# PlakarLabs/plakar

Hardware: AMD Instinct MI355X
Metric: GiB/s chunked (device-resident, cut-points out) at 1/2/4/8 MI355X (higher is better)
Workload: dtype u8; 1 GPU; C1: 1x 1 GiB uniform random buffer per GPU (BASELINE configs[1]); bytes_per_gpu=1073741824, global_bytes=1073741824, buffers_per_gpu=1, chunk_params=FASTCDC min 65536 / normal 1048576 / max 4194304, gear=placeholder (v0.0.8 table unavailable; see DESIGN.md), parallelism=independent buffers, 1 rank per GPU x 1, no collective, streams=2

## Files before the change

### include/plakar_cdc.h

```cpp
#ifndef PLAKAR_CDC_H
#define PLAKAR_CDC_H

#include <stddef.h>
#include <stdint.h>

#ifdef __cplusplus
extern "C" {
#endif

#define CDC_ABI_VERSION 1

#define CDC_OK 0
#define CDC_EOF 1
#define CDC_NEED_DATA 2
#define CDC_E_INVALID (-1)
#define CDC_E_UNSUPPORTED (-2)
#define CDC_E_NOSPACE (-3)
#define CDC_E_DEVICE (-4)
#define CDC_E_NOMEM (-5)
#define CDC_E_NORMAL_SIZE (-6)
#define CDC_E_MIN_SIZE (-7)
#define CDC_E_MAX_SIZE (-8)
#define CDC_E_IO (-9)
#define CDC_E_NOT_INIT (-10)
// ... 310 lines not shown
                             uint64_t host_min_len, void *stream, uint64_t *host_chunks, uint64_t *host_bytes);
int cdc_chunk_entropy_device_async(int device, const uint32_t *d_hist, uint64_t rows, double *d_entropy,
                                   void *stream);

typedef struct cdc_stream cdc_stream;
int cdc_stream_new(const char *algorithm, const cdc_opts *opts, uint64_t window_bytes, int device,
                   cdc_stream **out);
int cdc_stream_buffer(cdc_stream *s, uint8_t **write_ptr, uint64_t *space);
int cdc_stream_commit(cdc_stream *s, uint64_t nbytes, int eof);
int cdc_stream_next(cdc_stream *s, const uint8_t **chunk, uint64_t *len);
void cdc_stream_free(cdc_stream *s);

typedef int64_t (*cdc_read_fn)(void *ctx, void *buf, uint64_t cap);
typedef struct cdc_chunker cdc_chunker;
int cdc_chunker_new(const char *algorithm, cdc_read_fn read, void *ctx, const cdc_opts *opts,
                    cdc_chunker **out);
int cdc_chunker_next(cdc_chunker *c, const uint8_t **chunk, uint64_t *len);
void cdc_chunker_free(cdc_chunker *c);

int cdc_set_debug_mode(int mode);

int cdc_set_maskl_index_mode(int mode);

int cdc_debug_maskl_state(int device, uint32_t *hint, uint64_t *groups);

int cdc_debug_stream_read(int device, const void *d_buf, uint64_t len, int reps, double best_us[3], double median_us[3],
                          void *stream);

int cdc_debug_set_digest_lanes(uint64_t lanes);

int cdc_profile_enable(int on);
int cdc_profile_collect(double *scan_ms, double *pipeline_ms, uint64_t *launches,
                        uint64_t *scan_bytes);

#ifdef __cplusplus
}
#endif
#endif
```

### plakar_amd/_lib.py

```python
import ctypes
import os
import sys
import warnings

_HERE = os.path.dirname(os.path.abspath(__file__))
LIB_PATH = os.environ.get("PLAKAR_CDC_LIB") or os.path.join(_HERE, "_lib", "libplakar_cdc.so")

CDC_OK = 0
CDC_EOF = 1
CDC_NEED_DATA = 2
CDC_E_INVALID = -1
CDC_E_UNSUPPORTED = -2
CDC_E_NOSPACE = -3
CDC_E_DEVICE = -4
CDC_E_NOMEM = -5
CDC_E_NORMAL_SIZE = -6
CDC_E_MIN_SIZE = -7
CDC_E_MAX_SIZE = -8
CDC_E_IO = -9
CDC_E_NOT_INIT = -10
CDC_E_NO_DEVICE = -11
CDC_E_AUTH = -12
CDC_E_CORRUPT = -13
CDC_E_MISMATCH = -14
# ... 251 lines not shown
    "cdc_archive_new": (ctypes.c_int, [ctypes.c_int, _P(cdc_archive_opts), _P(ctypes.c_void_p)]),
    "cdc_archive_add_packfile": (ctypes.c_int, [ctypes.c_void_p, ctypes.c_void_p, ctypes.c_uint64]),
    "cdc_archive_add_packfile_path": (ctypes.c_int, [ctypes.c_void_p, ctypes.c_char_p]),
    "cdc_archive_run": (ctypes.c_int, [ctypes.c_void_p, _P(cdc_archive_entry), ctypes.c_int, ctypes.c_char_p,
                                       ARCHIVE_DATA_FN, ARCHIVE_ENTRY_FN, ctypes.c_void_p, _P(cdc_archive_stats)]),
    "cdc_archive_free": (None, [ctypes.c_void_p]),
    "cdc_set_debug_mode": (ctypes.c_int, [ctypes.c_int]),
    "cdc_gear_is_placeholder": (ctypes.c_int, []),
    "cdc_set_maskl_index_mode": (ctypes.c_int, [ctypes.c_int]),
    "cdc_backup_run": (ctypes.c_int, [ctypes.c_int, _P(ctypes.c_char_p), ctypes.c_int, _P(cdc_backup_opts),
                                      BACKUP_FILE_FN, BACKUP_PACK_FN, ctypes.c_void_p, _P(cdc_backup_stats)]),
    "cdc_backup_new": (ctypes.c_int, [ctypes.c_int, _P(cdc_backup_opts), _P(ctypes.c_void_p)]),
    "cdc_backup_files": (ctypes.c_int, [ctypes.c_void_p, _P(ctypes.c_char_p), ctypes.c_int, BACKUP_FILE_FN,
                                        BACKUP_PACK_FN, ctypes.c_void_p, _P(cdc_backup_stats)]),
    "cdc_backup_free": (None, [ctypes.c_void_p]),
    "cdc_sha256": (ctypes.c_int, [ctypes.c_void_p, ctypes.c_uint64, ctypes.c_int, _P(ctypes.c_uint8)]),
    "cdc_sha256_accelerated": (ctypes.c_int, []),
    "cdc_chunk_entropy_device_async": (ctypes.c_int, [ctypes.c_int, ctypes.c_void_p, ctypes.c_uint64, ctypes.c_void_p,
                                                      ctypes.c_void_p]),
    "cdc_debug_maskl_state": (ctypes.c_int, [ctypes.c_int, _P(ctypes.c_uint32), _P(ctypes.c_uint64)]),
    "cdc_debug_stream_read": (ctypes.c_int, [ctypes.c_int, ctypes.c_void_p, ctypes.c_uint64, ctypes.c_int,
                                             ctypes.c_double * 3, ctypes.c_double * 3, ctypes.c_void_p]),
    "cdc_debug_set_digest_lanes": (ctypes.c_int, [ctypes.c_uint64]),
    "cdc_profile_enable": (ctypes.c_int, [ctypes.c_int]),
    "cdc_profile_collect": (ctypes.c_int, [_P(ctypes.c_double), _P(ctypes.c_double),
                                           _P(ctypes.c_uint64), _P(ctypes.c_uint64)]),
}

_lib = None


def lib():
    global _lib
    if _lib is None:
        if not os.path.exists(LIB_PATH):
            raise ImportError(
                f"libplakar_cdc.so not found at {LIB_PATH}: the HIP extension is required "
                "(build it with `python -m plakar_amd.build`); there is no CPU fallback")
        torch = sys.modules.get("torch")
        if torch is not None:
            try:
                torch.cuda.is_available()
            except Exception:
                pass
        L = ctypes.CDLL(LIB_PATH)
        for name, (res, args) in SIGNATURES.items():
# ... 55 lines not shown
```

### plakar_amd/csrc/cdc_api.cpp

```cpp
#include <hip/hip_runtime.h>

#include <algorithm>
#include <chrono>
#include <cerrno>
#include <cctype>
#include <cstdio>
#include <cstdlib>
#include <cstring>
#include <atomic>
#include <condition_variable>
#include <functional>
#include <mutex>
#include <string>
#include <thread>
#include <vector>

#include <fcntl.h>
#include <sys/stat.h>
#include <unistd.h>

#include "cdc_hostmem.h"
#include "cdc_internal.h"

using namespace cdc;
// ... 9 lines not shown
    hipEvent_t staged = nullptr;
    hipEvent_t done = nullptr;
    uint8_t *d_in() const { return in.as<uint8_t>(); }
    cdc_cut *d_cuts() const { return cuts.as<cdc_cut>(); }
    cdc_cut *h_cuts() const { return cuts_h.as<cdc_cut>(); }
    cdc_result *d_res() const { return res.as<cdc_result>(); }
    cdc_result *h_res() const { return res_h.as<cdc_result>(); }
};

constexpr int kBounces = 2;

struct DeviceCtx {
    int device = -1;
    uint64_t *d_gear = nullptr;
    hipStream_t stream = nullptr;
    hipStream_t copy = nullptr;
    std::mutex mu;
    Slot slot[2];
    PinBuf bounce[kBounces];
    hipEvent_t bounce_ev[kBounces] = {nullptr, nullptr};
    int next_bounce = 0;
    uint32_t *hint_h = nullptr, *hint_d = nullptr;
    std::atomic<uint64_t> groups{0};
};

struct Global {
    std::mutex mu;
    std::atomic<bool> init{false};
    bool placeholder_gear = true;
    uint64_t gear[256];
    uint64_t mask_s = kDefaultMaskS, mask_l = kDefaultMaskL;
    uint32_t cut_adj = 0;
    int debug_mode = 0;
    std::vector<DeviceCtx *> devs;
};

Global &G()
{
    static Global g;
    return g;
}

std::atomic<uint32_t> &maskl_index_mode()
{
    static std::atomic<uint32_t> m([] {
        const char *e = getenv("CDC_MASKL_INDEX");
// ... 95 lines not shown

int grow_bounce(DeviceCtx *c, uint64_t bytes)
{
    if (c->bounce[kBounces - 1].data() && bytes <= c->bounce[kBounces - 1].cap()) return CDC_OK;
    HIPCHK(hipStreamSynchronize(c->copy));
    for (int k = 0; k < kBounces; ++k) {
        if (!c->bounce[k].reserve(bytes)) return CDC_E_DEVICE;
        if (!c->bounce_ev[k]) HIPCHK(hipEventCreateWithFlags(&c->bounce_ev[k], hipEventDisableTiming));
        HIPCHK(hipEventRecord(c->bounce_ev[k], c->copy));
    }
    return CDC_OK;
}

Workspace carve(void *ws, const Plan &pl, const uint64_t *gear)
{
    char *b = static_cast<char *>(ws);
    Workspace W;
    W.runs = reinterpret_cast<uint64_t *>(b + pl.off_runs);
    W.w1_nodes = reinterpret_cast<uint64_t *>(b + pl.off_w1_nodes);
    W.xg = reinterpret_cast<uint64_t *>(b + pl.off_xg);
    W.sg = reinterpret_cast<uint64_t *>(b + pl.off_sg);
    W.flags = reinterpret_cast<uint32_t *>(b + pl.off_flags);
    W.tick = reinterpret_cast<uint32_t *>(b + pl.off_tick);
    W.gear = gear;
    W.runsL = reinterpret_cast<uint64_t *>(b + pl.off_runsL);
    W.validL = reinterpret_cast<uint32_t *>(b + pl.off_validL);
    return W;
}

int run_group(DeviceCtx *ctx, const DevParams &P, const void *const *data, const uint64_t *lens,
              int n, int final_, cdc_cut *const *cuts, const uint64_t *caps,
              cdc_result *const *res, void *ws, uint64_t ws_bytes, void *stream)
{
    Plan pl;
    int st = make_plan(lens, n, P, &pl);
    if (st != CDC_OK) return st;
    if (ws_bytes < pl.bytes) return CDC_E_INVALID;
    Batch B;
    std::memset(&B, 0, sizeof(B));
    B.nbufs = uint32_t(n);
    B.final_ = final_ ? 1u : 0u;
    B.total_segs = pl.total_segs;
    B.total_tasks = pl.total_tasks;
    B.seg = pl.seg;
    B.scan_lane = pl.scan_lane;
    B.persist = pl.persist;
// ... 13 lines not shown
        volatile uint32_t *hint = ctx->hint_h;
        if (hint && k % 1024 == 1023) *hint = 0u;
        const bool hinted = !hint || *hint != 0u;
        B.maskl_index = mli >= 2 || (mli == 1 && hinted) ? 1u : 0u;
        B.maskl_fused = P.fm_ok && (mli == 2 || (mli == 1 && hinted)) ? 1u : 0u;
        B.maskl_probe = mli == 1 && !hinted && k % 16 == 0 ? 1u : 0u;
        B.maskl_hint = ctx->hint_d;
    }
    B.force_fallback = G().debug_mode == 1 ? 1u : 0u;
    uint32_t segs = 0, tasks = 0;
    for (int i = 0; i < n; ++i) {
        BufDesc &D = B.b[i];
        D.data = static_cast<const uint8_t *>(data[i]);
        D.len = lens[i];
        D.out = cuts[i];
        D.cap = caps[i];
        D.res = res[i];
        D.seg_base = segs;
        D.nseg = uint32_t((lens[i] + B.seg - 1) / B.seg);
        D.task_base = tasks;
        segs += D.nseg;
        tasks += uint32_t((lens[i] + 64ull * pl.scan_lane - 1) / (64ull * pl.scan_lane));
    }
    const Workspace W = carve(ws, pl, ctx->d_gear);
    return launch_batch(B, P, W, stream);
}

int group_ws_bytes(const uint64_t *lens, int n, const DevParams &P, uint64_t *bytes)
{
    Plan pl;
    const int st = make_plan(lens, n, P, &pl);
    if (st != CDC_OK) return st;
    *bytes = pl.bytes;
    return CDC_OK;
}

int check_ready(int device, DeviceCtx **out)
{
    Global &g = G();
    if (!g.init.load(std::memory_order_acquire)) return CDC_E_NOT_INIT;
    for (auto *c : g.devs)
        if (c->device == device) {
            *out = c;
            return CDC_OK;
        }
    return CDC_E_INVALID;
}
// ... 413 lines not shown
    if (!algorithm || !opts) return CDC_E_INVALID;
    const std::string a = lower(algorithm);
    if (a != "fastcdc") return CDC_E_UNSUPPORTED;
    return validate_sizes(opts);
}

int cdc_set_debug_mode(int mode)
{
    G().debug_mode = mode;
    return CDC_OK;
}

int cdc_set_maskl_index_mode(int mode)
{
    if (mode < 0 || mode > 3) return CDC_E_INVALID;
    maskl_index_mode().store(uint32_t(mode), std::memory_order_relaxed);
    Global &g = G();
    std::lock_guard<std::mutex> lock(g.mu);
    for (DeviceCtx *c : g.devs)
        if (c && c->hint_h) *static_cast<volatile uint32_t *>(c->hint_h) = 0u;
    return CDC_OK;
}

int cdc_debug_set_digest_lanes(uint64_t lanes)
{
    cdc::g_digest_lanes = lanes;
    return CDC_OK;
}

int cdc_debug_maskl_state(int device, uint32_t *hint, uint64_t *groups)
{
    if (!hint || !groups) return CDC_E_INVALID;
    DeviceCtx *ctx = nullptr;
    const int st = check_ready(device, &ctx);
    if (st != CDC_OK) return st;
    if (hipSetDevice(device) != hipSuccess || hipDeviceSynchronize() != hipSuccess) return CDC_E_DEVICE;
    *hint = ctx->hint_h ? *static_cast<volatile uint32_t *>(ctx->hint_h) : 1u;
    *groups = ctx->groups.load(std::memory_order_relaxed);
    return CDC_OK;
}

int cdc_debug_stream_read(int device, const void *d_buf, uint64_t len, int reps, double best_us[3], double median_us[3],
                          void *stream)
{
    if (!d_buf || !best_us || !median_us) return CDC_E_INVALID;
    DeviceCtx *ctx = nullptr;
    const int st = check_ready(device, &ctx);
    if (st != CDC_OK) return st;
    if (hipSetDevice(device) != hipSuccess) return CDC_E_DEVICE;
    return launch_stream_read(d_buf, len, reps, best_us, median_us, stream);
}

int cdc_device_count(void)
{
    int n = 0;
    if (hipGetDeviceCount(&n) != hipSuccess) return 0;
    return n;
}

static void destroy_ctx(DeviceCtx *c)
{
    (void)hipSetDevice(c->device);
    if (c->stream) (void)hipStreamSynchronize(c->stream);
    (void)hipDeviceSynchronize();
    if (c->hint_h) (void)hipHostFree(c->hint_h);
    if (c->d_gear) (void)hipFree(c->d_gear);
    if (c->copy) (void)hipStreamSynchronize(c->copy);
    free_ctx_buffers(c);
    if (c->stream) (void)hipStreamDestroy(c->stream);
    if (c->copy) (void)hipStreamDestroy(c->copy);
    delete c;
}

static int create_ctx(int d, DeviceCtx **out)
{
    auto *c = new DeviceCtx();
    c->device = d;
    *out = nullptr;
    if (hipSetDevice(d) != hipSuccess || hipStreamCreateWithFlags(&c->stream, hipStreamNonBlocking) != hipSuccess ||
        hipMalloc(reinterpret_cast<void **>(&c->d_gear), 256 * sizeof(uint64_t)) != hipSuccess) {
        destroy_ctx(c);
        return CDC_E_DEVICE;
    }
    if (hipHostMalloc(reinterpret_cast<void **>(&c->hint_h), 64, hipHostMallocMapped | hipHostMallocCoherent) ==
        hipSuccess) {
        *c->hint_h = 0u;
        if (hipHostGetDevicePointer(reinterpret_cast<void **>(&c->hint_d), c->hint_h, 0) != hipSuccess) {
            (void)hipHostFree(c->hint_h);
            c->hint_h = c->hint_d = nullptr;
        }
    }
    *out = c;
    return CDC_OK;
}

int cdc_init(uint32_t dev_mask, const uint64_t gear[256], uint64_t mask_s, uint64_t mask_l,
             int cut_convention)
{
    Global &g = G();
    std::lock_guard<std::mutex> lock(g.mu);
    if (cut_convention != 0 && cut_convention != 1) return CDC_E_INVALID;
    uint64_t tab[256];
    if (gear)
// ... 978 lines not shown
```

### plakar_amd/csrc/cdc_internal.h

```cpp
#pragma once

#include <stddef.h>
#include <stdint.h>

#include <vector>

#include "plakar_cdc.h"

namespace cdc {

constexpr int kMaxBufsPerLaunch = 32;
constexpr int64_t kRowPending = -0x7FF0;
constexpr uint32_t kDbgForceAbort = 512;
constexpr uint32_t kForceAbortTicks = 20000;
constexpr uint32_t kRunCap = 4;
constexpr uint32_t kRecCntBits = 8, kRecEntBits = 14;
constexpr uint32_t kMaxScanLane = 1u << kRecEntBits;
constexpr uint32_t kMaxSegs = 1u << 22;
constexpr uint32_t kScanLaneBytes = 16384;
#ifndef CDC_WALK_WAVES
#define CDC_WALK_WAVES 4
#endif
constexpr uint32_t kWalkWavesPerWG = CDC_WALK_WAVES;
constexpr uint64_t kUndet = ~0ull;
// ... 24 lines not shown
    uint32_t final_;
    uint32_t total_segs, total_tasks;
    uint32_t force_fallback;
    uint32_t scan_lane;
    uint32_t debug;
    uint32_t spin_ticks;
    uint32_t maskl_index;
    uint32_t maskl_fused;
    uint32_t *maskl_hint;
    uint32_t maskl_probe;
    uint64_t seg;
    uint32_t persist;
    uint32_t scan_wgs;
    BufDesc b[kMaxBufsPerLaunch];
};

struct Workspace {
    uint64_t *runs;
    uint64_t *w1_nodes;
    uint64_t *xg;
    uint64_t *sg;
    uint32_t *flags;
    uint32_t *tick;
    const uint64_t *gear;
    uint64_t *runsL;
    uint32_t *validL;
};

struct Plan {
    uint64_t seg;
    uint32_t scan_lane;
    uint32_t total_segs, total_tasks;
    uint32_t persist, scan_wgs;
    size_t off_runs, off_w1_nodes, off_xg, off_sg, off_flags, off_tick, off_runsL, off_validL,
        bytes;
};

int make_plan(const uint64_t *lens, int nbufs, const DevParams &P, Plan *plan);
int launch_batch(const Batch &B, const DevParams &P, const Workspace &W, void *stream);
struct DigestBuf {
    const uint8_t *data;
    uint64_t len;
    const cdc_cut *cuts;
    uint64_t cap;
    const cdc_result *res;
    uint8_t *digests;
// ... 71 lines not shown
```

### plakar_amd/csrc/cdc_kernels.hip

```cpp
#include <hip/hip_ext.h>
#include <hip/hip_runtime.h>

#include <algorithm>
#include <mutex>
#include <type_traits>
#include <vector>

#include "cdc_hostmem.h"
#include "cdc_internal.h"

namespace cdc {

#ifndef CDC_SPIN_SLEEP
#define CDC_SPIN_SLEEP 1
#endif
constexpr int kSpinSleep = CDC_SPIN_SLEEP;

static constexpr uint64_t kNoHit = ~0ull;
static constexpr uint32_t kRawLaneBytes = 512;
static constexpr uint32_t kWarm = 64;

template <int NT, int COPIES = 32>
__device__ __forceinline__ void fill_gear_lds(uint64_t *tab, const uint64_t *gear, uint32_t sh = 0)
{
// ... 289 lines not shown
        for (int j = 0; j < 4; ++j) {
            const uint64_t r0 = r4 + 64u * j;
            if (r0 > rb) break;
            const uint64_t E = __ballot(rec_cnt(rec[j]) == 0);
            const uint32_t n = uint32_t(min(rb + 1 - r0, uint64_t(64)));
            const uint64_t Z = ~E & (n == 64 ? ~0ull : (1ull << n) - 1);
            const uint64_t below = Z & ((1ull << lane) - 1);
            const uint32_t prev = below ? lane - 1u - (63u - uint32_t(__builtin_clzll(below))) : cur + lane;
            const uint64_t r = r0 + lane;
            bool need = false;
            if (lane < n) {
                if ((E >> lane) & 1ull)
                    need = r >= ra && prev + 1 >= kc;
                else
                    need = prev >= kc && r + kMaskLSpill >= ra;
            }
            if (__ballot(need)) return true;
            cur = Z ? n - 1u - (63u - uint32_t(__builtin_clzll(Z))) : cur + n;
        }
    }
    return false;
}

template <bool kMaskL, bool kFused>
__device__ __forceinline__ void scan_task(const Batch &B, const DevParams &P, const Workspace &W, char *s_lds,
                                          const char *tab, uint32_t task, uint32_t lane, uint32_t wave,
                                          uint32_t laneoff);

template <bool kMaskL, bool kFused = false>
__device__ __forceinline__ void scan_body(const Batch &B, const DevParams &P, const Workspace &W)
{
    static_assert(!(kMaskL && kFused), "k_scan_f builds both indexes, from the MaskS records' side");
    __shared__ __attribute__((aligned(16)))
    char s_lds[kGearLdsBytes + kS2Waves * (kStageBytes + kQBytes) + (kFused ? kFlushTabBytes : 0u)];
    const uint32_t lane = threadIdx.x & 63u;
    const uint32_t wave = __builtin_amdgcn_readfirstlane(threadIdx.x >> 6);
    const uint32_t laneoff = (lane & 31u) << 3;
    const uint32_t task = blockIdx.x * kS2Waves + wave;
    bool act = true;
    if constexpr (kMaskL) {
        act = false;
        if (task < B.total_tasks) {
            uint32_t bb = 0;
            while (bb + 1 < B.nbufs && task >= B.b[bb + 1].task_base) ++bb;
            const BufDesc &Db = B.b[bb];
            const uint64_t t = task - Db.task_base;
            if (t * 64ull * B.scan_lane < Db.len) act = maskl_needed(B, P, W, Db, t, lane);
            if (lane == 0) W.validL[task] = act ? 1u : 0u;
        }
        if (!__syncthreads_or(act ? 1 : 0)) return;
        if (threadIdx.x == 0 && B.maskl_hint)
            __hip_atomic_store(B.maskl_hint, 1u, __ATOMIC_RELAXED, __HIP_MEMORY_SCOPE_SYSTEM);
    }
    if constexpr (!kMaskL) {
        const uint32_t gt = blockIdx.x * blockDim.x + threadIdx.x, nth = gridDim.x * blockDim.x;
        for (uint32_t i = gt; i < B.total_segs; i += nth) {
            W.xg[i] = 0ull;
            W.sg[i] = 0ull;
        }
        if (gt < kMaxBufsPerLaunch + 4)
            W.flags[gt] = gt == kLimitWord ? uint32_t(B.spin_ticks ? B.spin_ticks : kSpinLimit) : 0u;
        if (gt < 2) W.tick[gt] = 0u;
        if (gt < B.nbufs) B.b[gt].res->status = kRowPending;
        if (threadIdx.x == 0) dbg_ts(B, kTsScan + 4 * blockIdx.x);
    }
    uint32_t clk = 0;
    if (!kMaskL && (B.debug & kDbgClk) && blockIdx.x == 0 && threadIdx.x == 0) {
        clk = kTsClk + 4u * uint32_t(atomicAdd(reinterpret_cast<unsigned long long *>(&g_ts[kTsClkN]), 1ull) % kClkRecs);
        g_ts[clk] = __builtin_amdgcn_s_memrealtime();
        g_ts[clk + 1] = __builtin_amdgcn_s_memtime();
    }
    fill_gear_lds<kS2Waves * 64>(reinterpret_cast<uint64_t *>(s_lds), W.gear,
                                 kFused ? P.fm_sh : kMaskL ? P.fl_sh : P.fs_sh);
    if constexpr (kFused) {
        static_assert(kS2Waves * 64 >= 256, "one entry per thread");
        if (threadIdx.x < 256)
            reinterpret_cast<uint64_t *>(s_lds + kGearLdsBytes + kS2Waves * (kStageBytes + kQBytes))[threadIdx.x] =
                W.gear[threadIdx.x] << P.fs_sh;
    }
    __syncthreads();
    if (!kMaskL && threadIdx.x == 0) {
        dbg_ts(B, kTsScan + 4 * blockIdx.x + 1);
        if (blockIdx.x < 4096)
            dbg_ts(B, kTsHw + blockIdx.x,
                   uint64_t(__builtin_amdgcn_s_getreg(20 | (0 << 6) | (15 << 11))) << 32 |
                       uint32_t(__builtin_amdgcn_s_getreg(4 | (0 << 6) | (31 << 11))));
    }
    const char *tab = s_lds;
    if (!act) return;
    const bool persist = !kMaskL && B.persist != 0;
    auto next_task = [&]() { return wave_ticket(W.tick + 2); };
    for (uint32_t cur = persist ? next_task() : task;;) {
        if (cur >= B.total_tasks) break;
        scan_task<kMaskL, kFused>(B, P, W, s_lds, tab, cur, lane, wave, laneoff);
        if (!persist) break;
        cur = next_task();
    }
    if (clk && threadIdx.x == 0) {
        g_ts[clk + 2] = __builtin_amdgcn_s_memrealtime();
        g_ts[clk + 3] = __builtin_amdgcn_s_memtime();
    }
}

template <bool kMaskL, bool kFused>
__device__ __forceinline__ void scan_task(const Batch &B, const DevParams &P, const Workspace &W, char *s_lds,
                                          const char *tab, uint32_t task, uint32_t lane, uint32_t wave,
                                          uint32_t laneoff)
{
    uint32_t b = 0;
    while (b + 1 < B.nbufs && task >= B.b[b + 1].task_base) ++b;
    const BufDesc &D = B.b[b];

    const uint64_t sl = B.scan_lane;
    const uint64_t ub = reinterpret_cast<uint64_t>(D.data);
    const uint64_t lo_ok = ub & ~15ull, hi_ok = (ub + D.len + 15) & ~15ull;
    const uint64_t seg0 = uint64_t(task - D.task_base) * 64u;
    if (seg0 * sl >= D.len) return;
    const int64_t s = int64_t((seg0 + lane) * sl);
    constexpr uint32_t kLead = 128u;
    const uint32_t T = uint32_t((sl + kLead + (ub & 15u) + kStage - 1u) / kStage);
    const uint64_t wb = ((ub + seg0 * sl) & ~15ull) - kLead;
    const uint64_t base = wb > lo_ok ? wb : lo_ok;
    const uint64_t limw = hi_ok - 16u - base;
    const uint32_t lim = limw > 0x7FFFFFFFull ? 0x7FFFFFFFu : uint32_t(limw);
    const uint32_t ring = uint32_t(reinterpret_cast<uintptr_t>(s_lds)) + kGearLdsBytes + wave * kStageBytes;
    static_assert(kStage == 64 && kL == 4, "pair staging: 64-B stages, one slot");
    const uint32_t half = lane >> 5;
    const uint32_t row = lane & 31u, swz = (row >> 1) & 7u;
    uint32_t offi[4];
    uint32_t om = 0;
#pragma unroll
    for (uint32_t j = 0; j < 4; ++j) {
        const uint32_t r = 8u * j + lane / 8u;
        const uint32_t k = (lane % 8u) ^ ((r >> 1) & 7u);
        const uint32_t o = uint32_t((((ub + (seg0 + r) * sl) & ~15ull) - kLead + 16u * k) - base);
        om = max(om, o);
        offi[j] = o - 1024u * j;
    }
    const uint64_t om0 = scan_wave_max(om);
    const uint64_t half_step = 32ull * sl;
    auto issue = [&](auto PC, uint32_t u, auto FC) {
        constexpr uint32_t Q = decltype(PC)::value;
        constexpr bool kFast = decltype(FC)::value;
        const uint64_t adv = uint64_t(kStage) * (u - Q) + (Q ? half_step : 0ull);
#ifdef CDC_DIAG_NO_DMA
        return;
#endif
        if (kFast || om0 + adv <= uint64_t(lim)) {
#ifdef CDC_DIAG_L2
            dma_stage_imm(lo_ok + ((base + adv - lo_ok) & 0x7FFF0ull), ring, offi);
#else
            dma_stage_imm(base + adv, ring, offi);
#endif
        } else {
            uint32_t eff[4];
#pragma unroll
            for (uint32_t j = 0; j < 4; ++j) eff[j] = min(offi[j] + 1024u * j + uint32_t(adv), lim);
            dma_stage(base, ring, eff);
        }
    };
    const char *rowp = s_lds + kGearLdsBytes + wave * kStageBytes + row * 128u;
    auto load_row = [&](uint4 (&first)[4], uint4 (&second)[4]) {
#ifdef CDC_DIAG_NO_ROW
        asm volatile("" : "+v"(first[0].x), "+v"(second[0].x));
        return;
#endif
#pragma unroll
        for (uint32_t g = 0; g < 4; ++g) first[g] = *reinterpret_cast<const uint4 *>(rowp + 16u * (g ^ swz));
#pragma unroll
        for (uint32_t g = 0; g < 4; ++g) second[g] = *reinterpret_cast<const uint4 *>(rowp + 16u * ((g + 4) ^ swz));
    };
    const uint32_t TT = T + 1;
    const int32_t lag = int32_t(kStage * half);
    const uint32_t vhi = to_vgpr(kFused ? P.fm_mi : kMaskL ? P.fl_hi : P.fs_hi);
    const uint32_t xlo = kMaskL ? P.fl_lo : P.fs_lo, xhi = kMaskL ? P.fl_hi : P.fs_hi;
    const int64_t rel0 = int64_t(((ub + uint64_t(s)) & ~15ull) - kLead) - int64_t(ub);
    using C0 = std::integral_constant<uint32_t, 0>;
    using C1 = std::integral_constant<uint32_t, 1>;
    using Gen = std::integral_constant<bool, false>;
    using Steady = std::integral_constant<bool, true>;

    uint4 A[4] = {}, Bv[4] = {};
#ifdef CDC_DIAG_WAITS
    uint64_t wsum = 0;
    uint32_t nrc = 0;
    const uint64_t tk0 = __builtin_amdgcn_s_memtime();
    const uint64_t rt0 = __builtin_amdgcn_s_memrealtime();
#endif
    static_assert(kLead >= 2 * kStage, "stage 0 must be pure warm-up for both halves");
    issue(C0{}, 0, Gen{});
    wait_vmcnt<0>();
    if (half == 0) load_row(A, Bv);
    asm volatile("s_waitcnt lgkmcnt(0)" ::: "memory");
    if (1 < TT) issue(C1{}, 1, Gen{});
    if (1 < TT) {
        wait_vmcnt<0>();
        if (half == 1) load_row(Bv, A);
        asm volatile("s_waitcnt lgkmcnt(0)" ::: "memory");
        if (2 < TT) issue(C0{}, 2, Gen{});
    }
    uint64_t gv[2][16];
#pragma unroll
    for (int k = 0; k < 16; ++k) gv[0][k] = lds_gear(tab, gear_addr(laneoff, word_of(Bv[0], k >> 2), k));
    uint64_t fp = 0;
    uint64_t rec = 0;
    uint64_t recL = 0;
    const int32_t rr0 = int32_t(rel0 - s) - lag;
    uint64_t *const qf = reinterpret_cast<uint64_t *>(s_lds + kGearLdsBytes + kS2Waves * kStageBytes + wave * kQBytes);
    uint32_t *const qm = reinterpret_cast<uint32_t *>(qf + kQCap);
    static_assert(kQCap == 64, "one flush pass: item j in lane j");
    uint32_t qn = 0;
    const char *const ftab = s_lds + kGearLdsBytes + kS2Waves * (kStageBytes + kQBytes);
    auto rgear = [&](const uint4 &d, int k) -> uint64_t {
        if constexpr (kFused)
            return lds_gear(ftab, __builtin_amdgcn_ubfe(word_of(d, k >> 2), uint32_t(k & 3) * 8u, 8u) << 3);
        else
            return lds_gear(tab, gear_addr(laneoff, word_of(d, k >> 2), k));
    };
    auto flush = [&]() {
        {
            const bool v = lane < qn;
            const uint32_t meta = qm[v ? lane : 0u];
            const uint32_t owner = meta >> 24;
            const int32_t r0 = int32_t(meta & 0xFFFFFFu) - 256;
            const int64_t so = int64_t((seg0 + owner) * sl);
            const int32_t ln = so < int64_t(D.len) ? int32_t(min(int64_t(sl), int64_t(D.len) - so)) : 0;
            const uint64_t a = ub + uint64_t(so + r0);
            auto clamp16 = [&](uint64_t x) { return min(max(x, lo_ok), hi_ok - 16u); };
            const uint4 d0 = gload16(clamp16(a)), d1 = gload16(clamp16(a + 16u));
            uint64_t f = 0;
            if constexpr (kFused) {
                uint4 dw[4];
#pragma unroll
                for (int h = 0; h < 4; ++h) dw[h] = gload16(clamp16(a - 64u + 16u * uint32_t(h)));
#pragma unroll
                for (int k = 0; k < 64; ++k) f = (f << 1) + rgear(dw[k >> 4], k & 15);
            } else {
                f = qf[v ? lane : 0u];
            }
            uint32_t miss = 0, missL = 0;
#pragma unroll
            for (int k = 0; k < 32; ++k) {
                f = (f << 1) + rgear(k < 16 ? d0 : d1, k & 15);
                miss |= min(key_of(f, xlo, xhi), 1u) << k;
                if constexpr (kFused) missL |= min(key_of(f, P.fm_llo, P.fm_lhi), 1u) << k;
            }
            const int32_t lo = r0 < 0 ? -r0 : 0, hi = ln - r0;
            uint32_t vm = lo >= 32 ? 0u : (0xFFFFFFFFu << lo);
            vm &= hi >= 32 ? 0xFFFFFFFFu : (hi <= 0 ? 0u : (1u << hi) - 1u);
// ... 40 lines not shown
            if ((gi & 1) == 0) {
                f0 = fp;
                acc = 0xFFFFFFFFu;
            }
#pragma unroll
            for (int q = 0; q < 4; ++q) {
#pragma unroll
                for (int k = 4 * q; k < 4 * q + 4; k += 2) {
                    const uint32_t a0 = gear_addr(laneoff, word_of(nx, k >> 2), k);
                    fp = (fp << 1) + cg[k];
                    ng[k] = lds_gear(tab, a0);
                    const uint32_t k0 = uint32_t(fp >> 32) & vhi;
                    const uint32_t a1 = gear_addr(laneoff, word_of(nx, (k + 1) >> 2), k + 1);
                    fp = (fp << 1) + cg[k + 1];
                    ng[k + 1] = lds_gear(tab, a1);
                    acc = umin3(acc, k0, uint32_t(fp >> 32) & vhi);
                    __builtin_amdgcn_sched_barrier(0);
                }
                __builtin_amdgcn_sched_barrier(0);
                if (q == 1 && gi + 1 == kGroups && (kSteady || t + 2 < TT)) {
                    asm volatile("s_waitcnt lgkmcnt(8)" ::: "memory");
                    issue(PC, t + 2, SC);
                    __builtin_amdgcn_sched_barrier(0);
                }
            }
            if (gi & 1) {
#ifndef CDC_DIAG_NO_RECHECK
                const uint64_t fm = __ballot(acc == 0);
#ifdef CDC_DIAG_WAITS
                nrc += fm ? 1u : 0u;
#endif
                if (fm) [[unlikely]] {
                    const uint32_t nq = uint32_t(__popcll(fm));
                    if (qn + nq > kQCap) flush();
                    if (acc == 0) {
                        const uint32_t idx =
                            qn + __builtin_amdgcn_mbcnt_hi(uint32_t(fm >> 32), __builtin_amdgcn_mbcnt_lo(uint32_t(fm), 0u));
                        const int32_t r0 = rr0 + int32_t(kStage * t + 16u * (gi - 1));
                        if constexpr (!kFused) qf[idx] = f0;
                        qm[idx] = uint32_t(r0 + 256) | (lane << 24);
                    }
                    qn += nq;
                }
#else
                rec += acc == 0 ? 1u : 0u;
#endif
            }
        }
    };
    if (1 < TT) stage(C1{}, Gen{}, 1, Bv, A);
    const int64_t room = int64_t(lim) - int64_t(om0) - int64_t(half_step);
    const int64_t tf = room >= 128 ? room / 64 - 1 : 0;
    const uint32_t t_steady = uint32_t(max<int64_t>(2, min<int64_t>(int64_t(TT) - 3, tf)));
    uint32_t t = 2;
    for (; t < t_steady; t += 2) {
        stage(C0{}, Steady{}, t, A, Bv);
        stage(C1{}, Steady{}, t + 1, Bv, A);
    }
    for (; t < TT; t += 2) {
        stage(C0{}, Gen{}, t, A, Bv);
        if (t + 1 < TT) stage(C1{}, Gen{}, t + 1, Bv, A);
    }
    if (qn) flush();
    if (s < int64_t(D.len)) (kMaskL ? W.runsL : W.runs)[64ull * D.task_base + seg0 + lane] = rec;
    if constexpr (kFused) {
        if (s < int64_t(D.len)) W.runsL[64ull * D.task_base + seg0 + lane] = recL;
        if (lane == 0) W.validL[task] = 1u;
    }
    if (!kMaskL && lane == 0) dbg_ts(B, kTsScan + 4 * blockIdx.x + 2 + (wave & 1));
#ifdef CDC_DIAG_WAITS
    if (lane == 0 && 8 * task + 7 < 8 * 16384) {
        uint64_t *o = g_ts + kTsRes + 8 * task;
        o[0] = wsum;
        o[1] = __builtin_amdgcn_s_memtime() - tk0;
        o[2] = rt0;
        o[3] = __builtin_amdgcn_s_memrealtime();
        o[4] = __builtin_amdgcn_s_getreg(4 | (0 << 6) | (31 << 11));
        o[5] = __builtin_amdgcn_s_getreg(20 | (0 << 6) | (15 << 11));
        o[6] = nrc;
        o[7] = wave;
    }
#endif
}

#ifndef CDC_SCAN_LB
#define CDC_SCAN_LB (kS2Waves * 64)
#endif
__global__ __launch_bounds__(CDC_SCAN_LB) void k_scan(const Batch B, const DevParams P, const Workspace W)
{
    scan_body<false>(B, P, W);
}

__global__ __launch_bounds__(kS2Waves * 64) void k_scan_l(const Batch B, const DevParams P, const Workspace W)
{
    scan_body<true>(B, P, W);
}

__global__ __launch_bounds__(CDC_SCAN_LB) void k_scan_f(const Batch B, const DevParams P, const Workspace W)
{
    scan_body<false, true>(B, P, W);
}

constexpr uint32_t kProbeWaves = 4;

__global__ __launch_bounds__(kProbeWaves * 64) void k_maskl_probe(const Batch B, const DevParams P, const Workspace W)
// ... 1086 lines not shown
            B.b[i].res->ncuts = 0;
            B.b[i].res->consumed = 0;
            B.b[i].res->needed = 0;
            if (B.total_tasks) settle_row(B.b[i].res, CDC_OK);
            else B.b[i].res->status = CDC_OK;
        }
    }
}

#ifdef CDC_RESOLVE_WAVES_PER_EU
#define CDC_RESOLVE_ATTR __attribute__((amdgpu_waves_per_eu(CDC_RESOLVE_WAVES_PER_EU)))
#else
#define CDC_RESOLVE_ATTR
#endif
__global__ CDC_RESOLVE_ATTR __launch_bounds__(kWalkWavesPerWG * 64) void k_resolve(const Batch B, const DevParams P, const Workspace W)
{
    __builtin_amdgcn_s_setprio(3);
    __shared__ uint64_t s_tab[256 * kWCopies];
    __shared__ uint64_t s_grec[kWalkWavesPerWG][kGRecs];
    __shared__ uint64_t s_gx[kWalkWavesPerWG][kGExtra];
    __shared__ uint32_t s_ticket;
    const uint32_t wave = threadIdx.x >> 6, lane = threadIdx.x & 63u;
    if (threadIdx.x == 0) s_ticket = __hip_atomic_fetch_add(W.tick, 1u, __ATOMIC_RELAXED, __HIP_MEMORY_SCOPE_AGENT);
    fill_gear_lds<kWalkWavesPerWG * 64, kWCopies>(s_tab, W.gear);
    __syncthreads();
    if (blockIdx.x == 0 && wave == 0) write_empty_rows(B, lane);
    const uint32_t g = uint32_t(__builtin_amdgcn_readfirstlane(s_ticket)) * kWalkWavesPerWG + wave;
    if (g < B.total_segs)
        resolve_segment(B, P, W, g, reinterpret_cast<const char *>(s_tab), graph_lds(s_grec[wave], s_gx[wave]));
}

constexpr uint32_t kStreamThreads = 256;

__global__ __launch_bounds__(kStreamThreads) void k_stream_read(const uint4 *p, uint64_t n16, uint32_t *sink)
{
    const uint64_t stride = uint64_t(gridDim.x) * kStreamThreads;
    uint64_t i = uint64_t(blockIdx.x) * kStreamThreads + threadIdx.x;
    uint32_t x = 0;
    for (; i + 3 * stride < n16; i += 4 * stride) {
        const uint4 a = p[i], b = p[i + stride], c = p[i + 2 * stride], d = p[i + 3 * stride];
        x ^= a.x ^ a.y ^ a.z ^ a.w ^ b.x ^ b.y ^ b.z ^ b.w ^ c.x ^ c.y ^ c.z ^ c.w ^ d.x ^ d.y ^ d.z ^ d.w;
    }
    for (; i < n16; i += stride) {
        const uint4 a = p[i];
        x ^= a.x ^ a.y ^ a.z ^ a.w;
    }
// ... 189 lines not shown
    if (!g_prof_on) return false;
    if (!g_prof_pool.empty()) {
        r = g_prof_pool.back();
        g_prof_pool.pop_back();
    } else if (hipEventCreate(&r.e0) != hipSuccess || hipEventCreate(&r.e1) != hipSuccess ||
               hipEventCreate(&r.e2) != hipSuccess) {
        return false;
    }
    r.scan_bytes = bytes;
    return true;
}

int launch_batch(const Batch &B, const DevParams &P, const Workspace &W, void *stream)
{
    hipStream_t st = reinterpret_cast<hipStream_t>(stream);
    if (B.nbufs == 0) return CDC_OK;
    uint64_t bytes = 0;
    for (uint32_t i = 0; i < B.nbufs; ++i) bytes += B.b[i].len;
    ProfRec pr;
    const bool prof = prof_begin(pr, bytes);
    const uint32_t need_wgs = (B.total_tasks + kS2Waves - 1) / kS2Waves;
    const dim3 sgrid(B.persist && B.scan_wgs < need_wgs ? B.scan_wgs : need_wgs), sblock(kS2Waves * 64);
    const bool fused = B.maskl_index && B.maskl_fused;
    if (B.persist && B.total_tasks > 0 && hipMemsetAsync(W.tick + 2, 0, 4, st) != hipSuccess) return CDC_E_DEVICE;
    if (B.total_tasks == 0) {
        if (prof) {
            (void)hipEventRecord(pr.e0, st);
            (void)hipEventRecord(pr.e1, st);
        }
    } else if (prof) {
        if (fused)
            hipExtLaunchKernelGGL(k_scan_f, sgrid, sblock, 0, st, pr.e0, pr.e1, 0, B, P, W);
        else
            hipExtLaunchKernelGGL(k_scan, sgrid, sblock, 0, st, pr.e0, pr.e1, 0, B, P, W);
    } else if (fused) {
        hipLaunchKernelGGL(k_scan_f, sgrid, sblock, 0, st, B, P, W);
    } else {
        hipLaunchKernelGGL(k_scan, sgrid, sblock, 0, st, B, P, W);
    }
#ifdef CDC_DIAG_SCAN_ONLY
    if (prof) {
        std::lock_guard<std::mutex> lk(g_prof_mu);
        (void)hipEventRecord(pr.e2, st);
        g_prof_live.push_back(pr);
    }
    return hipGetLastError() == hipSuccess ? CDC_OK : CDC_E_DEVICE;
#endif
// ... 88 lines not shown
```

### plakar_amd/device.py

```python
import ctypes

import torch

from . import _lib
from ._lib import check, ensure_init, lib


def _opts_c(opts):
    return _lib.cdc_opts(opts.MinSize, opts.NormalSize, opts.MaxSize, 0)


class DeviceBatch:

    def __init__(self, tensors, opts, final=True, device=None):
        ensure_init()
        if not tensors:
            raise ValueError("no buffers")
        self.tensors = list(tensors)
        for t in self.tensors:
            if t.dtype != torch.uint8 or not t.is_cuda or not t.is_contiguous():
                raise ValueError("expected contiguous uint8 CUDA tensors")
        self.device = self.tensors[0].device.index if device is None else device
        self.opts = opts
        self.final = 1 if final else 0
# ... 31 lines not shown
            ncuts, consumed, status, needed = (int(x) for x in r[i])
            check(status, f"buffer {i}")
            c = self.cuts[i][:ncuts].clone()
            c[:, 1] &= 0xFFFFFFFF
            out.append(c)
        return out, r


def chunk_device(tensors, opts, final=True):
    b = DeviceBatch(tensors, opts, final=final)
    b.launch()
    cuts, _ = b.results()
    return cuts


def set_debug_mode(mode):
    lib().cdc_set_debug_mode(int(mode))


def set_maskl_index_mode(mode):
    check(lib().cdc_set_maskl_index_mode(int(mode)))


def maskl_state(device=0):
    hint, groups = ctypes.c_uint32(), ctypes.c_uint64()
    check(lib().cdc_debug_maskl_state(int(device), ctypes.byref(hint), ctypes.byref(groups)))
    return hint.value, groups.value
```

Measured before the change: 5153 GiB/s.

## Prefetch next persistent scan task's DMA during current task tail and drop tick memset

Restructures the persistent scan loop so each wave claims its next task ticket during the current task's tail. It issues that task's first DMA stages before the flush and run writeback, which hides per-task warm-up latency. The scan ticket counter moves to a per-stream device slot that a later kernel resets, removing a hipMemsetAsync launch per call. The cost is more complex control flow, descriptor state carried across tasks, and a small per-stream lookup table. It also adds a debug setter for scan tasks per wave.

```diff
diff --git a/include/plakar_cdc.h b/include/plakar_cdc.h
--- a/include/plakar_cdc.h
+++ b/include/plakar_cdc.h
@@ -356,6 +356,8 @@
 
 int cdc_set_maskl_index_mode(int mode);
 
+int cdc_debug_set_scan_tasks_per_wave(int k);
+
 int cdc_debug_maskl_state(int device, uint32_t *hint, uint64_t *groups);
 
 int cdc_debug_stream_read(int device, const void *d_buf, uint64_t len, int reps, double best_us[3], double median_us[3],
diff --git a/plakar_amd/_lib.py b/plakar_amd/_lib.py
--- a/plakar_amd/_lib.py
+++ b/plakar_amd/_lib.py
@@ -297,6 +297,7 @@
     "cdc_debug_stream_read": (ctypes.c_int, [ctypes.c_int, ctypes.c_void_p, ctypes.c_uint64, ctypes.c_int,
                                              ctypes.c_double * 3, ctypes.c_double * 3, ctypes.c_void_p]),
     "cdc_debug_set_digest_lanes": (ctypes.c_int, [ctypes.c_uint64]),
+    "cdc_debug_set_scan_tasks_per_wave": (ctypes.c_int, [ctypes.c_int]),
     "cdc_profile_enable": (ctypes.c_int, [ctypes.c_int]),
     "cdc_profile_collect": (ctypes.c_int, [_P(ctypes.c_double), _P(ctypes.c_double),
                                            _P(ctypes.c_uint64), _P(ctypes.c_uint64)]),
diff --git a/plakar_amd/csrc/cdc_api.cpp b/plakar_amd/csrc/cdc_api.cpp
--- a/plakar_amd/csrc/cdc_api.cpp
+++ b/plakar_amd/csrc/cdc_api.cpp
@@ -55,6 +55,22 @@
     int next_bounce = 0;
     uint32_t *hint_h = nullptr, *hint_d = nullptr;
     std::atomic<uint64_t> groups{0};
+    static constexpr int kTickStreams = 16, kTickStride = 32;
+    uint32_t *scan_ticks = nullptr;
+    std::mutex tick_mu;
+    std::vector<void *> tick_streams;
+    uint32_t *scan_tick_of(void *stream)
+    {
+        if (!scan_ticks || stream == static_cast<void *>(hipStreamPerThread)) return nullptr;
+        std::lock_guard<std::mutex> lk(tick_mu);
+        size_t i = 0;
+        while (i < tick_streams.size() && tick_streams[i] != stream) ++i;
+        if (i == tick_streams.size()) {
+            if (i >= size_t(kTickStreams)) return nullptr;
+            tick_streams.push_back(stream);
+        }
+        return scan_ticks + i * kTickStride;
+    }
 };
 
 struct Global {
@@ -196,6 +212,8 @@
     W.sg = reinterpret_cast<uint64_t *>(b + pl.off_sg);
     W.flags = reinterpret_cast<uint32_t *>(b + pl.off_flags);
     W.tick = reinterpret_cast<uint32_t *>(b + pl.off_tick);
+    W.scan_tick = W.tick + 2;
+    W.scan_tick_armed = 0u;
     W.gear = gear;
     W.runsL = reinterpret_cast<uint64_t *>(b + pl.off_runsL);
     W.validL = reinterpret_cast<uint32_t *>(b + pl.off_validL);
@@ -255,7 +273,11 @@
         segs += D.nseg;
         tasks += uint32_t((lens[i] + 64ull * pl.scan_lane - 1) / (64ull * pl.scan_lane));
     }
-    const Workspace W = carve(ws, pl, ctx->d_gear);
+    Workspace W = carve(ws, pl, ctx->d_gear);
+    if (uint32_t *tk = ctx->scan_tick_of(stream)) {
+        W.scan_tick = tk;
+        W.scan_tick_armed = 1u;
+    }
     return launch_batch(B, P, W, stream);
 }
 
@@ -715,6 +737,13 @@
     return CDC_OK;
 }
 
+int cdc_debug_set_scan_tasks_per_wave(int k)
+{
+    if (k < -1 || k > 64) return CDC_E_INVALID;
+    cdc::t_scan_tpw = k;
+    return CDC_OK;
+}
+
 int cdc_debug_set_digest_lanes(uint64_t lanes)
 {
     cdc::g_digest_lanes = lanes;
@@ -758,6 +787,7 @@
     (void)hipDeviceSynchronize();
     if (c->hint_h) (void)hipHostFree(c->hint_h);
     if (c->d_gear) (void)hipFree(c->d_gear);
+    if (c->scan_ticks) (void)hipFree(c->scan_ticks);
     if (c->copy) (void)hipStreamSynchronize(c->copy);
     free_ctx_buffers(c);
     if (c->stream) (void)hipStreamDestroy(c->stream);
@@ -772,6 +802,12 @@
     *out = nullptr;
     if (hipSetDevice(d) != hipSuccess || hipStreamCreateWithFlags(&c->stream, hipStreamNonBlocking) != hipSuccess ||
         hipMalloc(reinterpret_cast<void **>(&c->d_gear), 256 * sizeof(uint64_t)) != hipSuccess) {
+        destroy_ctx(c);
+        return CDC_E_DEVICE;
+    }
+    const size_t tick_bytes = size_t(DeviceCtx::kTickStreams) * DeviceCtx::kTickStride * sizeof(uint32_t);
+    if (hipMalloc(reinterpret_cast<void **>(&c->scan_ticks), tick_bytes) != hipSuccess ||
+        hipMemset(c->scan_ticks, 0, tick_bytes) != hipSuccess) {
         destroy_ctx(c);
         return CDC_E_DEVICE;
     }
diff --git a/plakar_amd/csrc/cdc_internal.h b/plakar_amd/csrc/cdc_internal.h
--- a/plakar_amd/csrc/cdc_internal.h
+++ b/plakar_amd/csrc/cdc_internal.h
@@ -70,6 +70,8 @@
     uint64_t *sg;
     uint32_t *flags;
     uint32_t *tick;
+    uint32_t *scan_tick;
+    uint32_t scan_tick_armed;
     const uint64_t *gear;
     uint64_t *runsL;
     uint32_t *validL;
diff --git a/plakar_amd/csrc/cdc_kernels.hip b/plakar_amd/csrc/cdc_kernels.hip
--- a/plakar_amd/csrc/cdc_kernels.hip
+++ b/plakar_amd/csrc/cdc_kernels.hip
@@ -335,9 +335,97 @@
     return false;
 }
 
+struct ScanId {
+    uint32_t task, b;
+    uint32_t TT;
+    uint32_t t_steady;
+};
+struct ScanDma {
+    uint64_t base;
+    uint32_t lim;
+    uint32_t om0;
+    uint32_t offi[kL];
+#ifdef CDC_DIAG_L2
+    uint64_t lo_ok;
+#endif
+};
+
+constexpr uint32_t kScanLead = 128u;
+
+__device__ __forceinline__ bool scan_desc(const Batch &B, uint32_t task, uint32_t lane, ScanId &id, ScanDma &d)
+{
+    uint32_t b = 0;
+    while (b + 1 < B.nbufs && task >= B.b[b + 1].task_base) ++b;
+    const BufDesc &D = B.b[b];
+    const uint64_t sl = B.scan_lane;
+    const uint64_t ub = reinterpret_cast<uint64_t>(D.data);
+    const uint64_t lo_ok = ub & ~15ull, hi_ok = (ub + D.len + 15) & ~15ull;
+    const uint64_t seg0 = uint64_t(task - D.task_base) * 64u;
+    if (seg0 * sl >= D.len) return false;
+    id.task = task;
+    id.b = b;
+#ifdef CDC_DIAG_L2
+    d.lo_ok = lo_ok;
+#endif
+    const uint32_t T = uint32_t((sl + kScanLead + (ub & 15u) + kStage - 1u) / kStage);
+    const uint64_t wb = ((ub + seg0 * sl) & ~15ull) - kScanLead;
+    const uint64_t base = wb > lo_ok ? wb : lo_ok;
+    const uint64_t limw = hi_ok - 16u - base;
+    d.base = base;
+    d.lim = limw > 0x7FFFFFFFull ? 0x7FFFFFFFu : uint32_t(limw);
+    id.TT = T + 1;
+    uint32_t om = 0;
+#pragma unroll
+    for (uint32_t j = 0; j < kL; ++j) {
+        const uint32_t r = 8u * j + lane / 8u;
+        const uint32_t k = (lane % 8u) ^ ((r >> 1) & 7u);
+        const uint32_t o = uint32_t((((ub + (seg0 + r) * sl) & ~15ull) - kScanLead + 16u * k) - base);
+        om = max(om, o);
+        d.offi[j] = o - 1024u * j;
+    }
+    d.om0 = scan_wave_max(om);
+    const int64_t room = int64_t(d.lim) - int64_t(d.om0) - int64_t(32ull * sl);
+    const int64_t tf = room >= 128 ? room / 64 - 1 : 0;
+    id.t_steady = uint32_t(max<int64_t>(2, min<int64_t>(int64_t(id.TT) - 3, tf)));
+    return true;
+}
+
+template <uint32_t Q, bool kFast>
+__device__ __forceinline__ void scan_issue(const Batch &B, const ScanDma &d, uint32_t ring, uint32_t u)
+{
+    const uint64_t adv = uint64_t(kStage) * (u - Q) + (Q ? 32ull * B.scan_lane : 0ull);
+#ifdef CDC_DIAG_NO_DMA
+    return;
+#endif
+    if (kFast || uint64_t(d.om0) + adv <= uint64_t(d.lim)) {
+#ifdef CDC_DIAG_L2
+        dma_stage_imm(d.lo_ok + ((d.base + adv - d.lo_ok) & 0x7FFF0ull), ring, d.offi);
+#else
+        dma_stage_imm(d.base + adv, ring, d.offi);
+#endif
+    } else {
+        uint32_t eff[kL];
+#pragma unroll
+        for (uint32_t j = 0; j < kL; ++j) eff[j] = min(d.offi[j] + 1024u * j + uint32_t(adv), d.lim);
+        dma_stage(d.base, ring, eff);
+    }
+}
+
+__device__ __forceinline__ void scan_load_row(const char *rowp, uint32_t swz, uint4 (&first)[4], uint4 (&second)[4])
+{
+#ifdef CDC_DIAG_NO_ROW
+    asm volatile("" : "+v"(first[0].x), "+v"(second[0].x));
+    return;
+#endif
+#pragma unroll
+    for (uint32_t g = 0; g < 4; ++g) first[g] = *reinterpret_cast<const uint4 *>(rowp + 16u * (g ^ swz));
+#pragma unroll
+    for (uint32_t g = 0; g < 4; ++g) second[g] = *reinterpret_cast<const uint4 *>(rowp + 16u * ((g + 4) ^ swz));
+}
+
 template <bool kMaskL, bool kFused>
 __device__ __forceinline__ void scan_task(const Batch &B, const DevParams &P, const Workspace &W, char *s_lds,
-                                          const char *tab, uint32_t task, uint32_t lane, uint32_t wave,
+                                          const char *tab, ScanId cur, ScanDma dm, bool persist, uint32_t lane, uint32_t wave,
                                           uint32_t laneoff);
 
 template <bool kMaskL, bool kFused = false>
@@ -383,6 +471,18 @@
         g_ts[clk] = __builtin_amdgcn_s_memrealtime();
         g_ts[clk + 1] = __builtin_amdgcn_s_memtime();
     }
+    const bool persist = !kMaskL && B.persist != 0;
+    const uint32_t ring = uint32_t(reinterpret_cast<uintptr_t>(s_lds)) + kGearLdsBytes + wave * kStageBytes;
+    ScanId first;
+    ScanDma dm;
+    bool have = false;
+    if (act) {
+        for (uint32_t t0 = task; t0 < B.total_tasks; t0 = gridDim.x * kS2Waves + wave_ticket(W.scan_tick)) {
+            have = scan_desc(B, t0, lane, first, dm);
+            if (have || !persist) break;
+        }
+        if (have) scan_issue<0, false>(B, dm, ring, 0);
+    }
     fill_gear_lds<kS2Waves * 64>(reinterpret_cast<uint64_t *>(s_lds), W.gear,
                                  kFused ? P.fm_sh : kMaskL ? P.fl_sh : P.fs_sh);
     if constexpr (kFused) {
@@ -400,15 +500,7 @@
                        uint32_t(__builtin_amdgcn_s_getreg(4 | (0 << 6) | (31 << 11))));
     }
     const char *tab = s_lds;
-    if (!act) return;
-    const bool persist = !kMaskL && B.persist != 0;
-    auto next_task = [&]() { return wave_ticket(W.tick + 2); };
-    for (uint32_t cur = persist ? next_task() : task;;) {
-        if (cur >= B.total_tasks) break;
-        scan_task<kMaskL, kFused>(B, P, W, s_lds, tab, cur, lane, wave, laneoff);
-        if (!persist) break;
-        cur = next_task();
-    }
+    if (have) scan_task<kMaskL, kFused>(B, P, W, s_lds, tab, first, dm, persist, lane, wave, laneoff);
     if (clk && threadIdx.x == 0) {
         g_ts[clk + 2] = __builtin_amdgcn_s_memrealtime();
         g_ts[clk + 3] = __builtin_amdgcn_s_memtime();
@@ -417,108 +509,57 @@
 
 template <bool kMaskL, bool kFused>
 __device__ __forceinline__ void scan_task(const Batch &B, const DevParams &P, const Workspace &W, char *s_lds,
-                                          const char *tab, uint32_t task, uint32_t lane, uint32_t wave,
+                                          const char *tab, ScanId cur, ScanDma dm, bool persist, uint32_t lane, uint32_t wave,
                                           uint32_t laneoff)
 {
-    uint32_t b = 0;
-    while (b + 1 < B.nbufs && task >= B.b[b + 1].task_base) ++b;
-    const BufDesc &D = B.b[b];
-
+    constexpr uint32_t kLead = kScanLead;
     const uint64_t sl = B.scan_lane;
-    const uint64_t ub = reinterpret_cast<uint64_t>(D.data);
-    const uint64_t lo_ok = ub & ~15ull, hi_ok = (ub + D.len + 15) & ~15ull;
-    const uint64_t seg0 = uint64_t(task - D.task_base) * 64u;
-    if (seg0 * sl >= D.len) return;
-    const int64_t s = int64_t((seg0 + lane) * sl);
-    constexpr uint32_t kLead = 128u;
-    const uint32_t T = uint32_t((sl + kLead + (ub & 15u) + kStage - 1u) / kStage);
-    const uint64_t wb = ((ub + seg0 * sl) & ~15ull) - kLead;
-    const uint64_t base = wb > lo_ok ? wb : lo_ok;
-    const uint64_t limw = hi_ok - 16u - base;
-    const uint32_t lim = limw > 0x7FFFFFFFull ? 0x7FFFFFFFu : uint32_t(limw);
     const uint32_t ring = uint32_t(reinterpret_cast<uintptr_t>(s_lds)) + kGearLdsBytes + wave * kStageBytes;
     static_assert(kStage == 64 && kL == 4, "pair staging: 64-B stages, one slot");
     const uint32_t half = lane >> 5;
     const uint32_t row = lane & 31u, swz = (row >> 1) & 7u;
-    uint32_t offi[4];
-    uint32_t om = 0;
-#pragma unroll
-    for (uint32_t j = 0; j < 4; ++j) {
-        const uint32_t r = 8u * j + lane / 8u;
-        const uint32_t k = (lane % 8u) ^ ((r >> 1) & 7u);
-        const uint32_t o = uint32_t((((ub + (seg0 + r) * sl) & ~15ull) - kLead + 16u * k) - base);
-        om = max(om, o);
-        offi[j] = o - 1024u * j;
-    }
-    const uint64_t om0 = scan_wave_max(om);
-    const uint64_t half_step = 32ull * sl;
-    auto issue = [&](auto PC, uint32_t u, auto FC) {
-        constexpr uint32_t Q = decltype(PC)::value;
-        constexpr bool kFast = decltype(FC)::value;
-        const uint64_t adv = uint64_t(kStage) * (u - Q) + (Q ? half_step : 0ull);
-#ifdef CDC_DIAG_NO_DMA
-        return;
-#endif
-        if (kFast || om0 + adv <= uint64_t(lim)) {
-#ifdef CDC_DIAG_L2
-            dma_stage_imm(lo_ok + ((base + adv - lo_ok) & 0x7FFF0ull), ring, offi);
-#else
-            dma_stage_imm(base + adv, ring, offi);
-#endif
-        } else {
-            uint32_t eff[4];
-#pragma unroll
-            for (uint32_t j = 0; j < 4; ++j) eff[j] = min(offi[j] + 1024u * j + uint32_t(adv), lim);
-            dma_stage(base, ring, eff);
-        }
-    };
     const char *rowp = s_lds + kGearLdsBytes + wave * kStageBytes + row * 128u;
-    auto load_row = [&](uint4 (&first)[4], uint4 (&second)[4]) {
-#ifdef CDC_DIAG_NO_ROW
-        asm volatile("" : "+v"(first[0].x), "+v"(second[0].x));
-        return;
-#endif
-#pragma unroll
-        for (uint32_t g = 0; g < 4; ++g) first[g] = *reinterpret_cast<const uint4 *>(rowp + 16u * (g ^ swz));
-#pragma unroll
-        for (uint32_t g = 0; g < 4; ++g) second[g] = *reinterpret_cast<const uint4 *>(rowp + 16u * ((g + 4) ^ swz));
-    };
-    const uint32_t TT = T + 1;
+    auto load_row = [&](uint4 (&first)[4], uint4 (&second)[4]) { scan_load_row(rowp, swz, first, second); };
     const int32_t lag = int32_t(kStage * half);
     const uint32_t vhi = to_vgpr(kFused ? P.fm_mi : kMaskL ? P.fl_hi : P.fs_hi);
     const uint32_t xlo = kMaskL ? P.fl_lo : P.fs_lo, xhi = kMaskL ? P.fl_hi : P.fs_hi;
-    const int64_t rel0 = int64_t(((ub + uint64_t(s)) & ~15ull) - kLead) - int64_t(ub);
     using C0 = std::integral_constant<uint32_t, 0>;
     using C1 = std::integral_constant<uint32_t, 1>;
     using Gen = std::integral_constant<bool, false>;
     using Steady = std::integral_constant<bool, true>;
 
     uint4 A[4] = {}, Bv[4] = {};
+    static_assert(kLead >= 2 * kStage, "stage 0 must be pure warm-up for both halves");
+    static_assert(kLaneQuant + kLead >= 5 * kStage, "DMAs 0 to 2 of every task exist");
+    wait_vmcnt<0>();
+    if (half == 0) load_row(A, Bv);
+    asm volatile("s_waitcnt lgkmcnt(0)" ::: "memory");
+    scan_issue<1, false>(B, dm, ring, 1);
+    wait_vmcnt<0>();
+    if (half == 1) load_row(Bv, A);
+    asm volatile("s_waitcnt lgkmcnt(0)" ::: "memory");
+    scan_issue<0, false>(B, dm, ring, 2);
+  for (;;) {
+    const uint32_t task = cur.task, TT = cur.TT;
+    const int32_t rr0 = -int32_t((uint32_t(reinterpret_cast<uint64_t>(B.b[cur.b].data)) & 15u) + kLead) - lag;
+    auto issue = [&](auto PC, uint32_t u, auto FC) {
+        scan_issue<decltype(PC)::value, decltype(FC)::value>(B, dm, ring, u);
+    };
+    ScanId nxt;
+    bool has_next = false;
+    uint32_t ticket = 0;
 #ifdef CDC_DIAG_WAITS
     uint64_t wsum = 0;
     uint32_t nrc = 0;
     const uint64_t tk0 = __builtin_amdgcn_s_memtime();
     const uint64_t rt0 = __builtin_amdgcn_s_memrealtime();
 #endif
-    static_assert(kLead >= 2 * kStage, "stage 0 must be pure warm-up for both halves");
-    issue(C0{}, 0, Gen{});
-    wait_vmcnt<0>();
-    if (half == 0) load_row(A, Bv);
-    asm volatile("s_waitcnt lgkmcnt(0)" ::: "memory");
-    if (1 < TT) issue(C1{}, 1, Gen{});
-    if (1 < TT) {
-        wait_vmcnt<0>();
-        if (half == 1) load_row(Bv, A);
-        asm volatile("s_waitcnt lgkmcnt(0)" ::: "memory");
-        if (2 < TT) issue(C0{}, 2, Gen{});
-    }
     uint64_t gv[2][16];
 #pragma unroll
     for (int k = 0; k < 16; ++k) gv[0][k] = lds_gear(tab, gear_addr(laneoff, word_of(Bv[0], k >> 2), k));
     uint64_t fp = 0;
     uint64_t rec = 0;
     uint64_t recL = 0;
-    const int32_t rr0 = int32_t(rel0 - s) - lag;
     uint64_t *const qf = reinterpret_cast<uint64_t *>(s_lds + kGearLdsBytes + kS2Waves * kStageBytes + wave * kQBytes);
     uint32_t *const qm = reinterpret_cast<uint32_t *>(qf + kQCap);
     static_assert(kQCap == 64, "one flush pass: item j in lane j");
@@ -532,12 +573,16 @@
     };
     auto flush = [&]() {
         {
+            const BufDesc &D = B.b[cur.b];
+            const uint64_t ub = reinterpret_cast<uint64_t>(D.data), dlen = D.len;
+            const uint64_t lo_ok = ub & ~15ull, hi_ok = (ub + dlen + 15) & ~15ull;
+            const uint64_t seg0 = uint64_t(task - D.task_base) * 64u;
             const bool v = lane < qn;
             const uint32_t meta = qm[v ? lane : 0u];
             const uint32_t owner = meta >> 24;
             const int32_t r0 = int32_t(meta & 0xFFFFFFu) - 256;
             const int64_t so = int64_t((seg0 + owner) * sl);
-            const int32_t ln = so < int64_t(D.len) ? int32_t(min(int64_t(sl), int64_t(D.len) - so)) : 0;
+            const int32_t ln = so < int64_t(dlen) ? int32_t(min(int64_t(sl), int64_t(dlen) - so)) : 0;
             const uint64_t a = ub + uint64_t(so + r0);
             auto clamp16 = [&](uint64_t x) { return min(max(x, lo_ok), hi_ok - 16u); };
             const uint4 d0 = gload16(clamp16(a)), d1 = gload16(clamp16(a + 16u));
@@ -624,6 +669,18 @@
                     asm volatile("s_waitcnt lgkmcnt(8)" ::: "memory");
                     issue(PC, t + 2, SC);
                     __builtin_amdgcn_sched_barrier(0);
+                } else if (!kSteady && !kMaskL && q == 1 && gi + 1 == kGroups) {
+                    if (persist && t + 2 == TT) {
+                        asm volatile("s_waitcnt lgkmcnt(0)" ::: "memory");
+                        const uint32_t dyn0 = gridDim.x * kS2Waves;
+                        for (uint32_t nt = dyn0 + uint32_t(__builtin_amdgcn_readfirstlane(ticket)); nt < B.total_tasks;
+                             nt = dyn0 + wave_ticket(W.scan_tick)) {
+                            has_next = scan_desc(B, nt, lane, nxt, dm);
+                            if (has_next) break;
+                        }
+                        if (has_next) scan_issue<0, false>(B, dm, ring, 0);
+                        __builtin_amdgcn_sched_barrier(0);
+                    }
                 }
             }
             if (gi & 1) {
@@ -650,23 +707,35 @@
             }
         }
     };
-    if (1 < TT) stage(C1{}, Gen{}, 1, Bv, A);
-    const int64_t room = int64_t(lim) - int64_t(om0) - int64_t(half_step);
-    const int64_t tf = room >= 128 ? room / 64 - 1 : 0;
-    const uint32_t t_steady = uint32_t(max<int64_t>(2, min<int64_t>(int64_t(TT) - 3, tf)));
+    stage(C1{}, Gen{}, 1, Bv, A);
     uint32_t t = 2;
-    for (; t < t_steady; t += 2) {
+    for (; t < cur.t_steady; t += 2) {
         stage(C0{}, Steady{}, t, A, Bv);
         stage(C1{}, Steady{}, t + 1, Bv, A);
     }
+    if (!kMaskL && persist)
+        ticket = __hip_atomic_fetch_add(W.scan_tick, lane == 0u ? 1u : 0u, __ATOMIC_RELAXED, __HIP_MEMORY_SCOPE_AGENT);
     for (; t < TT; t += 2) {
         stage(C0{}, Gen{}, t, A, Bv);
         if (t + 1 < TT) stage(C1{}, Gen{}, t + 1, Bv, A);
     }
+    if (has_next) {
+        wait_vmcnt<0>();
+        if (half == 0) load_row(A, Bv);
+        asm volatile("s_waitcnt lgkmcnt(0)" ::: "memory");
+        scan_issue<1, false>(B, dm, ring, 1);
+    }
     if (qn) flush();
-    if (s < int64_t(D.len)) (kMaskL ? W.runsL : W.runs)[64ull * D.task_base + seg0 + lane] = rec;
+    if (has_next) {
+        wait_vmcnt<0>();
+        if (half == 1) load_row(Bv, A);
+        asm volatile("s_waitcnt lgkmcnt(0)" ::: "memory");
+        scan_issue<0, false>(B, dm, ring, 2);
+    }
+    const bool live = (uint64_t(task - B.b[cur.b].task_base) * 64u + lane) * sl < B.b[cur.b].len;
+    if (live) (kMaskL ? W.runsL : W.runs)[64ull * task + lane] = rec;
     if constexpr (kFused) {
-        if (s < int64_t(D.len)) W.runsL[64ull * D.task_base + seg0 + lane] = recL;
+        if (live) W.runsL[64ull * task + lane] = recL;
         if (lane == 0) W.validL[task] = 1u;
     }
     if (!kMaskL && lane == 0) dbg_ts(B, kTsScan + 4 * blockIdx.x + 2 + (wave & 1));
@@ -683,6 +752,9 @@
         o[7] = wave;
     }
 #endif
+    if (!has_next) break;
+    cur = nxt;
+  }
 }
 
 #ifndef CDC_SCAN_LB
@@ -1815,6 +1887,7 @@
     __shared__ uint32_t s_ticket;
     const uint32_t wave = threadIdx.x >> 6, lane = threadIdx.x & 63u;
     if (threadIdx.x == 0) s_ticket = __hip_atomic_fetch_add(W.tick, 1u, __ATOMIC_RELAXED, __HIP_MEMORY_SCOPE_AGENT);
+    if (blockIdx.x == 0 && threadIdx.x == 0) *W.scan_tick = 0u;
     fill_gear_lds<kWalkWavesPerWG * 64, kWCopies>(s_tab, W.gear);
     __syncthreads();
     if (blockIdx.x == 0 && wave == 0) write_empty_rows(B, lane);
@@ -2050,7 +2123,13 @@
     const uint32_t need_wgs = (B.total_tasks + kS2Waves - 1) / kS2Waves;
     const dim3 sgrid(B.persist && B.scan_wgs < need_wgs ? B.scan_wgs : need_wgs), sblock(kS2Waves * 64);
     const bool fused = B.maskl_index && B.maskl_fused;
-    if (B.persist && B.total_tasks > 0 && hipMemsetAsync(W.tick + 2, 0, 4, st) != hipSuccess) return CDC_E_DEVICE;
+#ifdef CDC_DIAG_SCAN_ONLY
+    const bool clear_tick = true;
+#else
+    const bool clear_tick = !W.scan_tick_armed;
+#endif
+    if (B.persist && B.total_tasks > 0 && clear_tick && hipMemsetAsync(W.scan_tick, 0, 4, st) != hipSuccess)
+        return CDC_E_DEVICE;
     if (B.total_tasks == 0) {
         if (prof) {
             (void)hipEventRecord(pr.e0, st);
diff --git a/plakar_amd/device.py b/plakar_amd/device.py
--- a/plakar_amd/device.py
+++ b/plakar_amd/device.py
@@ -77,6 +77,10 @@
     check(lib().cdc_set_maskl_index_mode(int(mode)))
 
 
+def set_scan_tasks_per_wave(k):
+    check(lib().cdc_debug_set_scan_tasks_per_wave(int(k)))
+
+
 def maskl_state(device=0):
     hint, groups = ctypes.c_uint32(), ctypes.c_uint64()
     check(lib().cdc_debug_maskl_state(int(device), ctypes.byref(hint), ctypes.byref(groups)))
```

Result: no change. 5207 GiB/s, median of 3 (+1.0%).
